# pangenome/impg

Measured on AMD Instinct MI355X. Metric: projected ranges/sec, 1M-PAF 100k-BED -x depth 3; CPU coitrees baseline, higher is better.
Workload: dtype int32

## Files before the change

### impg_amd/csrc/kernels.hip

```cpp
#include <hip/hip_runtime.h>

#include <cstring>
#include <type_traits>

#include "device_prims.hpp"
#include "impg_internal.hpp"
#include "kernels.hpp"

namespace impg {

__device__ __forceinline__ unsigned lane_id() { return threadIdx.x & 63u; }
__device__ __forceinline__ unsigned long long lanemask_lt() { return (1ull << lane_id()) - 1ull; }

template <int CTRL, int ROW_MASK>
__device__ __forceinline__ uint32_t dpp_or0(uint32_t x) {
  return (uint32_t)__builtin_amdgcn_update_dpp(0, (int)x, CTRL, ROW_MASK, 0xF, false);
}
__device__ __forceinline__ uint32_t wave_incl_scan(uint32_t x) {
  x += dpp_or0<0x111, 0xF>(x);
  x += dpp_or0<0x112, 0xF>(x);
  x += dpp_or0<0x114, 0xF>(x);
  x += dpp_or0<0x118, 0xF>(x);
  x += dpp_or0<0x142, 0xA>(x);
  x += dpp_or0<0x143, 0xC>(x);
// ... 2172 lines not shown
      const int sdir = reversed_entry ? 1 : (is_reverse ? -1 : 1);
      const int pdir = reversed_entry ? (is_reverse ? -1 : 1) : 1;
      const int32_t s0 = reversed_entry ? m_ts : (is_reverse ? m_te : m_ts);
      const int32_t p0 = reversed_entry ? (is_reverse ? m_qe : m_qs) : m_qs;
      const int64_t x_lo = sdir > 0 ? (int64_t)rs - s0 : (int64_t)s0 - re, x_hi = sdir > 0 ? (int64_t)re - s0 : (int64_t)s0 - rs;
      auto S = [&](uint32_t k) -> int64_t { const uint4 b = B[k]; return (int64_t)(reversed_entry ? b.y : b.x); };
      uint32_t lo = 1, hi = n + 1;
      while (lo < hi) { const uint32_t mid = (lo + hi) >> 1; if (S(mid) <= x_lo) lo = mid + 1; else hi = mid; }
      const uint32_t first = lo - 1;
      lo = 0; hi = n;
      while (lo < hi) { const uint32_t mid = (lo + hi) >> 1; if (S(mid) < x_hi) lo = mid + 1; else hi = mid; }
      if (first < n && lo > 0 && first <= lo - 1) {
        const uint32_t last = lo - 1;
        const uint4 bf0 = B[first], bf1 = B[first + 1], bl0 = B[last], bl1 = B[last + 1];
        auto seg = [&](const uint4 &a, const uint4 &b, int32_t &ppos, int32_t &pdelta, int32_t &sstart, int32_t &send, int32_t &asd) {
          const int32_t sa = (int32_t)(reversed_entry ? a.y : a.x), sb = (int32_t)(reversed_entry ? b.y : b.x);
          const int32_t ja = (int32_t)(reversed_entry ? a.x : a.y), jb = (int32_t)(reversed_entry ? b.x : b.y);
          const int32_t pa = s0 + sdir * sa, pb = s0 + sdir * sb;
          sstart = min(pa, pb); send = max(pa, pb); asd = sb - sa;
          ppos = p0 + pdir * ja; pdelta = pdir * (jb - ja);
        };
        const int32_t qlo = min(m_qs, m_qe), qhi = max(m_qs, m_qe);
        int32_t ppos, pdelta, sstart, send, asd;
        seg(bf0, bf1, ppos, pdelta, sstart, send, asd);
        const int32_t refined_first = tp_refine(ppos, pdelta, sstart, max(sstart, rs), asd, true, qlo, qhi);
        seg(bl0, bl1, ppos, pdelta, sstart, send, asd);
        const int32_t refined_last = tp_refine(ppos, pdelta, sstart, min(send, re), asd, false, qlo, qhi);
        bool keep = true;
        int64_t mm = 0, xx = 0;
        if (CIGAR || use_ident) { mm = (int64_t)bl1.z - bf0.z; xx = (int64_t)bl1.w - bf0.w; }
        if (use_ident) {
          const int64_t total = mm + xx;
          const double ident = total == 0 ? 0.0 : (double)mm / (double)total;
          keep = !(ident < min_identity);
        }
        if (keep) {
          if (refined_first < 0 || refined_last < 0) atomicOr(err_flag, 2u);
          const bool swap_q = is_reverse && !reversed_entry;
          out = make_int4(swap_q ? refined_last : refined_first, swap_q ? refined_first : refined_last, rs, re);
          qid = e1.x;
          ok = true;
          if (CIGAR) {
            const bool fits = mm <= (int64_t)OP_LEN_MASK && xx <= (int64_t)OP_LEN_MASK;
            if (!fits) atomicOr(err_flag, 4u);
            sl.a[p] = (uint32_t)mm;
            sl.off[p] = (int32_t)xx;
            sl.n[p] = fits ? (mm > 0 ? 1u : 0u) + (xx > 0 ? 1u : 0u) : 0u;
            sl.rem[p] = 0;
          }
        }
      }
    }
    h.qid[p] = qid;
    if (ok) h.c[p] = out;
  }
  __shared__ uint32_t wcnt[4];
  unsigned long long m = __ballot(ok);
  if (lane_id() == 0) wcnt[threadIdx.x >> 6] = __popcll(m);
  __syncthreads();
  if (threadIdx.x == 0) {
    uint32_t tot = wcnt[0] + wcnt[1] + wcnt[2] + wcnt[3];
    if (tot) atomicAdd(&accepted[(blockIdx.x % COUNT_SLOTS) * COUNT_STRIDE], (unsigned long long)tot);
  }
}

__global__ __launch_bounds__(256) void slice_counts_kernel(HitArrays h, SliceArrays sl, uint32_t n_pairs,
                                                           uint32_t *__restrict__ cnt) {
  const uint32_t p = blockIdx.x * 256u + threadIdx.x;
  if (p >= n_pairs) return;
  cnt[p] = h.qid[p] == HIT_NONE ? 0u : sl.n[p];
}
__global__ __launch_bounds__(64) void slice_write_kernel(DeviceIndexView v, const uint32_t *__restrict__ pair_entry,
                                                         HitArrays h, SliceArrays sl, uint32_t n_pairs,
                                                         const uint32_t *__restrict__ off, uint32_t *__restrict__ out) {
  const uint32_t p = blockIdx.x * 64u + threadIdx.x;
  if (p >= n_pairs || h.qid[p] == HIT_NONE) return;
  const Entry &en = v.entries[pair_entry[p]];
  const bool swp = (en.nops_flags & EF_REVERSED) != 0, flip = swp && (en.nops_flags & EF_STRAND);
  const uint32_t *rec = v.ops + (size_t)en.tile_base * TILE_WORDS;
  const uint32_t n = sl.n[p], a = sl.a[p];
  uint32_t *o = out + off[p];
  for (uint32_t t = 0; t < n; t++) {
    const uint32_t oi = flip ? a - t : a + t;
    uint32_t op = rec[(size_t)(oi / TILE_OPS) * TILE_WORDS + 6 + oi % TILE_OPS];
    if (swp) {
      const uint32_t code = op >> 29;
      if (code == 2u) op = (3u << 29) | (op & OP_LEN_MASK);
      else if (code == 3u) op = (2u << 29) | (op & OP_LEN_MASK);
    }
    o[t] = op;
  }
  const int32_t fo = sl.off[p], lr = sl.rem[p];
  if (fo > 0) o[0] = (o[0] & (7u << 29)) | (uint32_t)((int32_t)(o[0] & OP_LEN_MASK) - fo);
  if (lr < 0) o[n - 1] = (o[n - 1] & (7u << 29)) | (uint32_t)((int32_t)(o[n - 1] & OP_LEN_MASK) + lr);
}

__global__ __launch_bounds__(256) void slice_write_tp_kernel(HitArrays h, SliceArrays sl, uint32_t n_pairs,
                                                             const uint32_t *__restrict__ off, uint32_t *__restrict__ out) {
  const uint32_t p = blockIdx.x * 256u + threadIdx.x;
  if (p >= n_pairs || h.qid[p] == HIT_NONE || sl.n[p] == 0u) return;
  const uint32_t mm = sl.a[p], xx = (uint32_t)sl.off[p];
  uint32_t *o = out + off[p];
  if (mm) *o++ = mm | (0u << 29);
  if (xx) *o = xx | (1u << 29);
}

__device__ __forceinline__ unsigned long long mix64(unsigned long long z) {
  z = (z ^ (z >> 30)) * 0xBF58476D1CE4E5B9ull;
  z = (z ^ (z >> 27)) * 0x94D049BB133111EBull;
  return z ^ (z >> 31);
}
__global__ __launch_bounds__(256) void hit_stats_kernel(const FrontierRec *__restrict__ fr,
                                                        const uint32_t *__restrict__ pair_range, uint32_t n_pairs,
                                                        HitArrays h, int32_t min_output_length, int skip_same_target,
                                                        unsigned long long *__restrict__ rstat, int want_ck, uint32_t stride) {
  const uint32_t p = blockIdx.x * 256u + threadIdx.x;
  uint32_t r = 0xFFFFFFFFu;
  unsigned long long c = 0, a = 0;
  if (p < n_pairs) {
    r = pair_range[(size_t)p * stride];
    const uint32_t qid = h.qid[(size_t)p * stride];
    if (qid != HIT_NONE) {
      const uint32_t tgt = fr[r].target_id;
      const int4 hc = h.c[p];
      const int32_t qs = hc.x, qe = hc.y;
      const bool drop = (min_output_length >= 0 && abs(qe - qs) < min_output_length) ||
                        (skip_same_target && qid == tgt);
      if (!drop) {
        if (want_ck) {
          a = mix64(((unsigned long long)qid << 32) | (uint32_t)qs);
          a = mix64(a ^ (((unsigned long long)(uint32_t)qe << 32) | tgt));
          a = mix64(a ^ (((unsigned long long)(uint32_t)hc.z << 32) | (uint32_t)hc.w));
        }
        c = 1;
      }
    }
  }
  const unsigned lane = lane_id();
  const uint32_t prev = (uint32_t)__shfl_up((int)r, 1);
  const unsigned long long heads = __ballot(lane == 0 || prev != r);
  if (__popcll(heads) < 64) {
    const unsigned first = 63u - (unsigned)__clzll((long long)(heads & (lanemask_lt() | (1ull << lane))));
#pragma unroll
    for (unsigned o = 1; o < 64; o <<= 1) {
      const unsigned long long cv = (unsigned long long)__shfl_up((long long)c, o);
      const unsigned long long av = (unsigned long long)__shfl_up((long long)a, o);
      if (lane >= first + o) { c += cv; a += av; }
    }
  }
  const bool tail = lane == 63u || ((heads >> (lane + 1u)) & 1ull);
  if (tail && c && r != 0xFFFFFFFFu) {
    atomicAdd(&rstat[2u * (size_t)r], c);
    if (want_ck) atomicAdd(&rstat[2u * (size_t)r + 1u], a);
  }
}
__global__ __launch_bounds__(256) void range_stats_reduce_kernel(const FrontierRec *__restrict__ fr, uint32_t n_fr,
                                                                 const unsigned long long *__restrict__ rstat,
                                                                 unsigned long long *__restrict__ count,
                                                                 unsigned long long *__restrict__ cksum) {
  const uint32_t i = blockIdx.x * 256u + threadIdx.x;
  uint32_t q = 0xFFFFFFFFu;
  unsigned long long c = 0, a = 0;
  if (i < n_fr) {
    q = fr[i].qidx;
    const ulonglong2 x = reinterpret_cast<const ulonglong2 *>(rstat)[i];
    c = x.x; a = x.y;
  }
  const unsigned lane = lane_id();
  const uint32_t prev = (uint32_t)__shfl_up((int)q, 1);
  const unsigned long long heads = __ballot(lane == 0 || prev != q);
  const unsigned first = 63u - (unsigned)__clzll((long long)(heads & (lanemask_lt() | (1ull << lane))));
#pragma unroll
  for (unsigned o = 1; o < 64; o <<= 1) {
    const unsigned long long cv = (unsigned long long)__shfl_up((long long)c, o);
    const unsigned long long av = (unsigned long long)__shfl_up((long long)a, o);
    if (lane >= first + o) { c += cv; a += av; }
  }
  const bool tail = lane == 63u || ((heads >> (lane + 1u)) & 1ull);
  if (tail && q != 0xFFFFFFFFu && (c | a)) {
    if (count && c) atomicAdd(&count[q], c);
    if (cksum && a) atomicAdd(&cksum[q], a);
  }
}

__global__ __launch_bounds__(256) void update_keys_kernel(const FrontierRec *__restrict__ fr,
                                                          const uint32_t *__restrict__ pair_range, uint32_t n_pairs,
                                                          HitArrays h, unsigned long long *__restrict__ keys,
                                                          unsigned long long *__restrict__ vals,
                                                          unsigned long long *__restrict__ n_active) {
  const uint32_t p = blockIdx.x * 256u + threadIdx.x;
  unsigned long long k = ~0ull;
  if (p < n_pairs) {
    const uint32_t qid = h.qid[p];
    unsigned long long v = 0;
    if (qid != HIT_NONE) {
      const FrontierRec f = fr[pair_range[p]];
      if (qid != f.target_id) {
        k = ((unsigned long long)f.qidx << 32) | qid;
        const int4 hc = h.c[p];
        v = ((unsigned long long)(uint32_t)min(hc.x, hc.y) << 32) | (uint32_t)max(hc.x, hc.y);
      }
    }
    keys[p] = k;
    vals[p] = v;
  }
  __shared__ uint32_t wcnt[4];
  unsigned long long m = __ballot(k != ~0ull);
  if (lane_id() == 0) wcnt[threadIdx.x >> 6] = __popcll(m);
  __syncthreads();
  if (threadIdx.x == 0) {
    uint32_t tot = wcnt[0] + wcnt[1] + wcnt[2] + wcnt[3];
    if (tot) atomicAdd(&n_active[(blockIdx.x % COUNT_SLOTS) * COUNT_STRIDE], (unsigned long long)tot);
  }
}

__global__ __launch_bounds__(256) void group_heads_kernel(const unsigned long long *__restrict__ skeys, uint32_t n,
                                                          uint32_t *__restrict__ head) {
  const uint32_t i = blockIdx.x * 256u + threadIdx.x;
  if (i >= n) return;
  const unsigned long long k = skeys[i];
  head[i] = (k != ~0ull) && (i == 0 || skeys[i - 1] != k);
}
__global__ __launch_bounds__(256) void group_scatter_kernel(const unsigned long long *__restrict__ skeys, uint32_t n,
                                                            const uint32_t *__restrict__ head,
                                                            const uint32_t *__restrict__ gid,
                                                            uint32_t *__restrict__ gstart,
                                                            unsigned long long *__restrict__ gkey) {
  const uint32_t i = blockIdx.x * 256u + threadIdx.x;
  if (i >= n) return;
  if (head[i]) {
    gstart[gid[i]] = i;
    gkey[gid[i]] = skeys[i];
  }
}

constexpr uint32_t GROUP_ITEMS = 8, GROUP_TILE = 256u * GROUP_ITEMS;
__global__ __launch_bounds__(256) void group_count_kernel(const unsigned long long *__restrict__ skeys, uint32_t n, uint32_t *__restrict__ tile_heads) {
  const uint32_t base = blockIdx.x * GROUP_TILE + threadIdx.x * GROUP_ITEMS;
  unsigned long long prev = base > 0 && base <= n ? skeys[base - 1u] : 0ull;
  uint32_t c = 0;
#pragma unroll
  for (uint32_t k = 0; k < GROUP_ITEMS; k++) {
    const uint32_t i = base + k;
    const unsigned long long key = i < n ? skeys[i] : ~0ull;
    c += (key != ~0ull && (i == 0 || key != prev)) ? 1u : 0u;
    prev = key;
  }
  uint32_t tot;
  block_excl_scan(c, &tot);
  if (threadIdx.x == 0) tile_heads[blockIdx.x] = tot;
}
__global__ __launch_bounds__(256) void group_fill_kernel(const unsigned long long *__restrict__ skeys, uint32_t n, const uint32_t *__restrict__ tile_base,
                                                         uint32_t *__restrict__ gstart, unsigned long long *__restrict__ gkey) {
  const uint32_t base = blockIdx.x * GROUP_TILE + threadIdx.x * GROUP_ITEMS;
  unsigned long long key[GROUP_ITEMS];
  unsigned long long prev = base > 0 && base <= n ? skeys[base - 1u] : 0ull;
  uint32_t c = 0, flags = 0;
#pragma unroll
  for (uint32_t k = 0; k < GROUP_ITEMS; k++) {
    const uint32_t i = base + k;
    key[k] = i < n ? skeys[i] : ~0ull;
    if (key[k] != ~0ull && (i == 0 || key[k] != prev)) { flags |= 1u << k; c += 1u; }
    prev = key[k];
  }
  uint32_t tot;
  uint32_t g = tile_base[blockIdx.x] + block_excl_scan(c, &tot);
#pragma unroll
  for (uint32_t k = 0; k < GROUP_ITEMS; k++)
    if (flags & (1u << k)) { gstart[g] = base + k; gkey[g] = key[k]; g += 1u; }
}

constexpr uint32_t SEG_MAX_SEQ = 2048, SEG_WAVES = 4;
constexpr uint32_t SEG_BIG_QUERY = 32768;
constexpr uint32_t SEG_SLICE_HITS = 8192, SEG_BIG_SLICE = 131072, SEG_MAX_PARTS = 4096;
__global__ __launch_bounds__(256) void run_bounds_kernel(const uint32_t *__restrict__ pair_range, uint32_t n, uint32_t *__restrict__ run_start,
                                                         uint32_t *__restrict__ run_end) {
  const uint32_t p = blockIdx.x * 256u + threadIdx.x;
  if (p >= n) return;
  const uint32_t r = pair_range[p];
  if (p == 0 || pair_range[p - 1u] != r) run_start[r] = p;
  if (p + 1u == n || pair_range[p + 1u] != r) run_end[r] = p + 1u;
}
__global__ __launch_bounds__(256) void run_bounds_by_offsets_kernel(const uint32_t *__restrict__ perm, const uint32_t *__restrict__ pair_off,
                                                                    const uint32_t *__restrict__ cnt, uint32_t n_fr,
                                                                    uint32_t *__restrict__ run_start, uint32_t *__restrict__ run_end) {
  const uint32_t i = blockIdx.x * 256u + threadIdx.x;
  if (i >= n_fr) return;
  const uint32_t r = perm ? perm[i] : i, a = pair_off[i];
  run_start[r] = a;
  run_end[r] = a + cnt[i];
}
__global__ __launch_bounds__(256) void query_bounds_kernel(const FrontierRec *__restrict__ fr, uint32_t n_fr, uint32_t n_queries, uint32_t *__restrict__ qfirst,
                                                           uint32_t *__restrict__ qlast, uint32_t *__restrict__ unsorted) {
  const uint32_t i = blockIdx.x * 256u + threadIdx.x;
  if (i >= n_fr) return;
  const uint32_t q = fr[i].qidx;
  if (q >= n_queries) { *unsorted = 1u; return; }
  if (i == 0 || fr[i - 1u].qidx != q) {
    qfirst[q] = i;
    if (i && fr[i - 1u].qidx > q) *unsorted = 1u;
  }
  if (i + 1u == n_fr || fr[i + 1u].qidx != q) qlast[q] = i + 1u;
}
template <bool WITH_HC, class F>
__device__ __forceinline__ void seg_for_chunks(const FrontierRec *__restrict__ fr, const uint32_t *__restrict__ run_start,
                                               const uint32_t *__restrict__ run_end, const HitArrays &h, uint32_t f0, uint32_t f1, F f) {
  const uint32_t lane = lane_id();
  for (uint32_t base = f0; base < f1; base += 64u) {
    const uint32_t i = base + lane;
    const bool have = i < f1;
    const uint32_t rs = have ? run_start[i] : 0u, re = have ? run_end[i] : 0u, tg = have ? fr[i].target_id : 0u;
    const uint32_t m = min(64u, f1 - base);
    uint32_t j = 0, c0 = 0, e = 0, t = 0;
    auto seek = [&](uint32_t &jj, uint32_t &cc, uint32_t &ee, uint32_t &tt) {
      while (jj < m && cc >= ee) {
        jj += 1u;
        if (jj < m) {
          cc = (uint32_t)__builtin_amdgcn_readlane((int)rs, (int)jj);
          ee = (uint32_t)__builtin_amdgcn_readlane((int)re, (int)jj);
          tt = (uint32_t)__builtin_amdgcn_readlane((int)tg, (int)jj);
        }
      }
    };
    c0 = (uint32_t)__builtin_amdgcn_readlane((int)rs, 0);
    e = (uint32_t)__builtin_amdgcn_readlane((int)re, 0);
    t = (uint32_t)__builtin_amdgcn_readlane((int)tg, 0);
    seek(j, c0, e, t);
    uint32_t qid = HIT_NONE;
    int4 hc = make_int4(0, 0, 0, 0);
    if (j < m && c0 + lane < e) { qid = h.qid[c0 + lane]; if (WITH_HC) hc = h.c[c0 + lane]; }
    while (j < m) {
      uint32_t nj = j, nc = c0 + 64u, ne = e, nt = t;
      seek(nj, nc, ne, nt);
      uint32_t nqid = HIT_NONE;
      int4 nhc = make_int4(0, 0, 0, 0);
      if (nj < m && nc + lane < ne) { nqid = h.qid[nc + lane]; if (WITH_HC) nhc = h.c[nc + lane]; }
      f(qid, hc, qid != HIT_NONE && qid != t);
      j = nj; c0 = nc; e = ne; t = nt; qid = nqid; hc = nhc;
    }
  }
}
template <bool COUNT_ONLY>
__global__ __launch_bounds__(64 * SEG_WAVES) void seg_group_kernel(const FrontierRec *__restrict__ fr, const uint32_t *__restrict__ qfirst,
                                                                   const uint32_t *__restrict__ qlast, const uint32_t *__restrict__ run_start,
                                                                   const uint32_t *__restrict__ run_end, HitArrays h, uint32_t n_queries, uint32_t nb,
                                                                   uint32_t nbits, uint32_t *__restrict__ qact, const uint32_t *__restrict__ qdst,
                                                                   uint32_t *__restrict__ qgrp, const uint32_t *__restrict__ gdst,
                                                                   uint32_t *__restrict__ gstart, unsigned long long *__restrict__ gkey,
                                                                   unsigned long long *__restrict__ svals, uint32_t *__restrict__ qbins,
                                                                   uint32_t parts, uint32_t *__restrict__ qtot) {
  extern __shared__ __attribute__((aligned(16))) uint32_t seg_bins[];
  const uint32_t w = threadIdx.x >> 6, lane = lane_id();
  const uint32_t u = blockIdx.x * SEG_WAVES + w;
  if (u >= n_queries * parts) return;
  const bool sliced = parts > 1u;
  const uint32_t q = sliced ? u / parts : u, part = u - q * parts;
  uint32_t f0 = qfirst[q], f1 = qlast[q];
  if (sliced) {
    const uint32_t len = f1 > f0 ? f1 - f0 : 0u;
    f1 = f0 + (uint32_t)(((unsigned long long)len * (part + 1u)) / parts);
    f0 = f0 + (uint32_t)(((unsigned long long)len * part) / parts);
  } else if (f0 >= f1) { if (COUNT_ONLY && lane == 0) { qact[q] = 0u; qgrp[q] = 0u; } return; }
  uint32_t *bins = seg_bins + w * nb;
  if (COUNT_ONLY || !qbins) {
    for (uint32_t b = lane; b < nb; b += 64u) bins[b] = 0u;
    __builtin_amdgcn_wave_barrier();
    seg_for_chunks<false>(fr, run_start, run_end, h, f0, f1, [&](uint32_t qid, const int4 &, bool active) { if (active) atomicAdd(&bins[qid], 1u); });
  } else if (!sliced) {
    for (uint32_t b = lane; b < nb; b += 64u) bins[b] = qbins[(size_t)q * nb + b];
  }
  __builtin_amdgcn_wave_barrier();
  if (COUNT_ONLY) {
    uint32_t cnt = 0, grp = 0;
    for (uint32_t b = lane; b < nb; b += 64u) {
      const uint32_t x = bins[b];
      cnt += x; grp += x ? 1u : 0u;
      if (qbins) qbins[(size_t)u * nb + b] = x;
    }
#pragma unroll
    for (int o = 32; o > 0; o >>= 1) { cnt += (uint32_t)__shfl_xor((int)cnt, o); grp += (uint32_t)__shfl_xor((int)grp, o); }
    if (lane == 0) {
      if (!sliced) { qact[q] = cnt; qgrp[q] = grp; }
      if (cnt > (sliced ? SEG_BIG_SLICE : SEG_BIG_QUERY)) atomicMax(qact + 4u * (size_t)n_queries + 1u, cnt);
    }
    return;
  }
  const uint32_t dst0 = qdst[q];
  const unsigned long long khi = (unsigned long long)q << 32;
  uint32_t carry = 0, g = gdst[q];
  for (uint32_t b = 0; b < nb; b += 64u) {
    const uint32_t x = sliced ? qtot[(size_t)q * nb + b + lane] : bins[b + lane];
    const uint32_t inc = wave_incl_scan(x);
    const uint32_t off = carry + inc - x;
    bins[b + lane] = off + (sliced ? qbins[(size_t)u * nb + b + lane] : 0u);
    carry += (uint32_t)__builtin_amdgcn_readlane((int)inc, 63);
    const unsigned long long gm = __ballot(x != 0u);
    if (x && part == 0u) {
      const uint32_t gi = g + (uint32_t)__popcll(gm & lanemask_lt());
      gstart[gi] = dst0 + off;
      gkey[gi] = khi | (b + lane);
    }
    g += (uint32_t)__popcll(gm);
  }
  __builtin_amdgcn_wave_barrier();
  seg_for_chunks<true>(fr, run_start, run_end, h, f0, f1, [&](uint32_t qid, const int4 &hc, bool active) {
    const unsigned long long am = __ballot(active);
    if (!am) return;
    unsigned long long mask = am;
    for (uint32_t b = 0; b < nbits; b++) {
      const bool bit = (qid >> b) & 1u;
      const unsigned long long bal = __ballot(active && bit);
      mask &= bit ? bal : ~bal;
    }
    if (active) {
      const uint32_t pos = dst0 + bins[qid] + (uint32_t)__popcll(mask & lanemask_lt());
      svals[pos] = ((unsigned long long)(uint32_t)min(hc.x, hc.y) << 32) | (uint32_t)max(hc.x, hc.y);
    }
    __builtin_amdgcn_wave_barrier();
    if (active && lane == 63u - (uint32_t)__clzll((long long)mask)) bins[qid] += (uint32_t)__popcll(mask);
    __builtin_amdgcn_wave_barrier();
  });
}

__global__ __launch_bounds__(256) void seg_parts_scan_kernel(uint32_t *__restrict__ qbins, uint32_t nb, uint32_t parts, uint32_t *__restrict__ qtot,
                                                             uint32_t *__restrict__ qact, uint32_t *__restrict__ qgrp) {
  const uint32_t q = blockIdx.x, b = blockIdx.y * 256u + threadIdx.x;
  uint32_t run = 0;
  if (b < nb) {
    uint32_t *p = qbins + (size_t)q * parts * nb + b;
    uint32_t k = 0;
    for (; k + 4u <= parts; k += 4u) {
      const uint32_t x0 = p[(size_t)k * nb], x1 = p[(size_t)(k + 1u) * nb], x2 = p[(size_t)(k + 2u) * nb], x3 = p[(size_t)(k + 3u) * nb];
      p[(size_t)k * nb] = run; run += x0;
      p[(size_t)(k + 1u) * nb] = run; run += x1;
      p[(size_t)(k + 2u) * nb] = run; run += x2;
      p[(size_t)(k + 3u) * nb] = run; run += x3;
    }
    for (; k < parts; k++) { const uint32_t x = p[(size_t)k * nb]; p[(size_t)k * nb] = run; run += x; }
    qtot[(size_t)q * nb + b] = run;
  }
  uint32_t cnt = run, grp = run ? 1u : 0u;
#pragma unroll
  for (int o = 32; o > 0; o >>= 1) { cnt += (uint32_t)__shfl_xor((int)cnt, o); grp += (uint32_t)__shfl_xor((int)grp, o); }
  if (lane_id() == 0 && cnt) { atomicAdd(&qact[q], cnt); atomicAdd(&qgrp[q], grp); }
}

__device__ __forceinline__ uint32_t lower_bound_u64(const unsigned long long *a, uint32_t n, unsigned long long k) {
  uint32_t lo = 0, hi = n;
  while (lo < hi) {
    uint32_t mid = (lo + hi) >> 1;
    if (a[mid] < k) lo = mid + 1; else hi = mid;
  }
  return lo;
}

__global__ __launch_bounds__(256) void table_qoff_kernel(const unsigned long long *__restrict__ keys, uint32_t n_groups, uint32_t n_queries,
                                                         uint32_t *__restrict__ qoff) {
  const uint32_t q = blockIdx.x * 256u + threadIdx.x;
  if (q <= n_queries) qoff[q] = lower_bound_u64(keys, n_groups, (unsigned long long)q << 32);
}
__global__ __launch_bounds__(256) void group_prepare_kernel(VisitedTables vt, const unsigned long long *__restrict__ gkey,
                                                            const uint32_t *__restrict__ gstart, uint32_t n_groups,
                                                            uint32_t n_active, uint32_t *__restrict__ glen,
                                                            const int2 **__restrict__ old_src,
                                                            uint32_t *__restrict__ cap, uint32_t *__restrict__ pcap) {
  const uint32_t g = blockIdx.x * 256u + threadIdx.x;
  if (g >= n_groups) return;
  const uint32_t st = gstart[g];
  const uint32_t en = g + 1 < n_groups ? gstart[g + 1] : n_active;
  const uint32_t len = en - st;
  glen[g] = len;
  const unsigned long long k = gkey[g];
  const int2 *src = nullptr;
  uint32_t olen = 0;
  bool found = false;
  const uint32_t q = (uint32_t)(k >> 32);
  for (int t = (int)vt.n_tables - 1; t >= 0; t--) {
    const VisitedTable &T = vt.t[t];
    const uint32_t lo = T.qoff[q], hi = T.qoff[q + 1u];
    const uint32_t i = lo + lower_bound_u64(T.keys + lo, hi - lo, k);
    if (i < hi && T.keys[i] == k) {
      src = T.ranges + T.off[i];
      olen = T.len[i];
      found = true;
      break;
    }
  }
  if (!found && vt.mask_off) {
    const uint32_t seq = (uint32_t)(k & 0xFFFFFFFFull);
    const uint32_t a = vt.mask_off[seq];
    olen = vt.mask_off[seq + 1] - a;
    src = vt.mask_ranges + a;
  }
  old_src[g] = olen ? src : nullptr;
  cap[g] = olen + len;
  pcap[g] = olen + 2u * len;
}

__device__ __forceinline__ uint32_t lower_bound_start(const int2 *a, uint32_t n, int32_t s) {
  uint32_t lo = 0, hi = n;
  while (lo < hi) {
    uint32_t mid = (lo + hi) >> 1;
    if (a[mid].x < s) lo = mid + 1; else hi = mid;
  }
  return lo;
}

#ifndef IMPG_VU_LDS_CAP
#define IMPG_VU_LDS_CAP 12
#endif
constexpr uint32_t VU_LDS_CAP = IMPG_VU_LDS_CAP;
#ifndef IMPG_VW_TINY
#define IMPG_VW_TINY 192
#endif
#ifndef IMPG_VW_SMALL
#define IMPG_VW_SMALL 1152
#endif
#ifndef IMPG_VU_TINY_MAX
#define IMPG_VU_TINY_MAX 12
#endif
#ifndef IMPG_VU_MID_MAX
#define IMPG_VU_MID_MAX 48
#endif
#ifndef IMPG_VU_MID_CAP
#define IMPG_VU_MID_CAP 64
#endif
constexpr uint32_t VU_TINY_MAX = IMPG_VU_TINY_MAX, VU_MID_MAX = IMPG_VU_MID_MAX, VU_MID_CAP = IMPG_VU_MID_CAP;
static_assert(VU_TINY_MAX <= VU_LDS_CAP && VU_MID_MAX <= VU_MID_CAP, "a lane's list must fit its LDS column");
constexpr uint32_t VW_CAP_TINY = IMPG_VW_TINY, VW_CAP_SMALL = IMPG_VW_SMALL, VW_CAP_LARGE = 4096,
                   VW_SMALL_HEADROOM = 256;
struct ListInPlace {
  int2 *p;
  __device__ __forceinline__ int32_t &x(uint32_t i) const { return p[i].x; }
  __device__ __forceinline__ int32_t &y(uint32_t i) const { return p[i].y; }
};
struct ListInLds {
  int32_t *bx, *by;
  __device__ __forceinline__ int32_t &x(uint32_t i) const { return bx[i * 64u]; }
  __device__ __forceinline__ int32_t &y(uint32_t i) const { return by[i * 64u]; }
};
template <class L> __device__ __forceinline__ uint32_t list_lower_bound(const L &R, uint32_t n, int32_t s) {
  uint32_t lo = 0, hi = n;
  while (lo < hi) {
    const uint32_t mid = (lo + hi) >> 1;
    if (R.x(mid) < s) lo = mid + 1; else hi = mid;
  }
  return lo;
}
template <class L, class E, class G>
__device__ __forceinline__ void replay_one(const L &R, uint32_t &len, int32_t start, int32_t end, int32_t sequence_length,
                                           int32_t min_transitive_len, int32_t mdbr, E &&emit, G &&grow) {
  bool should_add = true;
  if (mdbr > 0) {
    const uint32_t idx = list_lower_bound(R, len, start);
    if (idx > 0 && abs(start - R.y(idx - 1)) < mdbr) should_add = false;
    if (should_add && idx < len && abs(R.x(idx) - end) < mdbr) should_add = false;
  }
  if (!should_add) return;
  if (start < 0) start = 0;
  if (end > sequence_length) end = sequence_length;
  int32_t current = start;
  const uint32_t pos = list_lower_bound(R, len, start);
  uint32_t i = pos;
  if (i > 0 && R.y(i - 1) > start) i -= 1;
  while (i < len && current < end) {
    const int32_t rx = R.x(i), ry = R.y(i);
    if (rx > end) break;
    if (current < rx) {
      if (abs(rx - current) >= min_transitive_len) emit(current, rx);
    }
    current = max(current, ry);
    i += 1;
  }
  if (current < end) {
    if (abs(end - current) >= min_transitive_len) emit(current, end);
  }
  uint32_t mfrom;
  if (pos > 0 && R.y(pos - 1) >= start) {
    R.y(pos - 1) = max(R.y(pos - 1), end);
    mfrom = pos - 1;
  } else if (pos < len && end >= R.x(pos)) {
    R.x(pos) = min(start, R.x(pos));
    R.y(pos) = max(end, R.y(pos));
    mfrom = pos;
  } else {
    grow();
    for (uint32_t k = len; k > pos; k--) { R.x(k) = R.x(k - 1); R.y(k) = R.y(k - 1); }
    R.x(pos) = start;
    R.y(pos) = end;
    len += 1;
    return;
  }
  uint32_t write = mfrom, read = mfrom + 1;
  while (read < len) {
    if (R.y(write) >= R.x(read)) {
      R.y(write) = max(R.y(write), R.y(read));
    } else {
      write += 1;
      const int32_t tx = R.x(write), ty = R.y(write);
      R.x(write) = R.x(read); R.y(write) = R.y(read);
      R.x(read) = tx; R.y(read) = ty;
    }
    read += 1;
  }
  len = write + 1;
}
template <class L>
__device__ __forceinline__ uint32_t replay_hits(const L &R, uint32_t len, const unsigned long long *__restrict__ svals,
                                                uint32_t st, uint32_t n, int32_t sequence_length,
                                                int32_t min_transitive_len, int32_t mdbr, int2 *__restrict__ P, uint32_t &np) {
  for (uint32_t t = 0; t < n; t++) {
    const unsigned long long iv = svals[st + t];
    replay_one(R, len, (int32_t)(uint32_t)(iv >> 32), (int32_t)(uint32_t)iv, sequence_length, min_transitive_len, mdbr,
               [&](int32_t a, int32_t b) { P[np++] = make_int2(a, b); }, [] {});
  }
  return len;
}
#ifdef IMPG_VU_CLOCKS
constexpr uint32_t VU_CLK_ROWS = 1024;
__device__ unsigned long long g_vu_clk[VU_CLK_ROWS][16];
#define VU_MARK(i) do { asm volatile("s_waitcnt vmcnt(0) lgkmcnt(0)" ::: "memory"); vu_t[i] = __builtin_readcyclecounter(); } while (0)
#else
#define VU_MARK(i) do { } while (0)
#endif
typedef const unsigned long long __attribute__((address_space(1))) *global_list_t;
__device__ __forceinline__ int2 list_range(global_list_t p, uint32_t i) {
  const unsigned long long v = p[i];
  return make_int2((int32_t)(uint32_t)v, (int32_t)(uint32_t)(v >> 32));
}
#ifndef IMPG_VU_WAVES
#define IMPG_VU_WAVES 6
#endif
#pragma clang diagnostic push
#pragma clang diagnostic ignored "-Wpass-failed"
template <uint32_t CAP, bool LISTED>
__global__ __launch_bounds__(64) __attribute__((amdgpu_waves_per_eu(IMPG_VU_WAVES, IMPG_VU_WAVES)))
void visited_update_kernel(const unsigned long long *__restrict__ svals,
                                                            const int32_t *__restrict__ seq_len,
                                                            const unsigned long long *__restrict__ gkey,
                                                            const uint32_t *__restrict__ gstart,
                                                            const uint32_t *__restrict__ glen,
                                                            const unsigned long long *__restrict__ old_src,
                                                            const uint32_t *__restrict__ cap,
                                                            const uint32_t *__restrict__ noff,
                                                            const uint32_t *__restrict__ poff, uint32_t n_groups,
                                                            int32_t min_transitive_len, int32_t mdbr,
                                                            int2 *__restrict__ new_ranges, uint32_t *__restrict__ new_len,
                                                            int2 *__restrict__ pieces, uint32_t *__restrict__ n_pieces,
                                                            const uint32_t *__restrict__ list, const uint32_t *__restrict__ n_list,
                                                            uint32_t *__restrict__ reach) {
  __shared__ int32_t lds_x[CAP * 64], lds_y[CAP * 64];
  const uint32_t n_items = LISTED ? *n_list : n_groups;
  for (uint32_t item0 = blockIdx.x * 64u; item0 < n_items; item0 += gridDim.x * 64u) {
  const uint32_t item = item0 + threadIdx.x;
#ifdef IMPG_VU_CLOCKS
  unsigned long long vu_t[8];
  VU_MARK(0);
#endif
  const bool have = item < n_items;
  const uint32_t g = LISTED ? list[min(item, n_items - 1u)] : item;
  const uint32_t gi = min(g, n_groups - 1u);
  const uint32_t c_ = cap[gi], n_ = glen[gi], st_ = gstart[gi], no = noff[gi], po = poff[gi];
  const global_list_t src_ = (global_list_t)old_src[gi];
  const unsigned long long key = gkey[gi];
  const uint32_t c = have ? c_ : 0u;
  const bool mine = have && (LISTED || c <= VU_TINY_MAX);
  const uint32_t n = mine ? n_ : 0u, st = mine ? st_ : 0u;
  const uint32_t olen = mine ? c - n : 0u;
  int2 *R = new_ranges + no;
  int2 *P = pieces + po;
  VU_MARK(1);
  const int32_t sequence_length = seq_len[(uint32_t)(key & 0xFFFFFFFFull)];
  const unsigned long long *hp = svals + st;
  const uint32_t hl = max(n, 1u) - 1u;
  unsigned long long h0 = hp[0], h1 = hp[min(1u, hl)], h2 = hp[min(2u, hl)], h3 = hp[min(3u, hl)];
  const global_list_t src = olen ? src_ : (global_list_t)(unsigned long long)(uintptr_t)svals;
  const uint32_t sl = max(olen, 1u) - 1u;
  const int2 s0 = list_range(src, 0), s1 = list_range(src, min(1u, sl)), s2 = list_range(src, min(2u, sl)), s3 = list_range(src, min(3u, sl));
  VU_MARK(2);
  uint32_t len = olen, np = 0;
  VU_MARK(3);
  const bool fast = mine;
  const ListInLds A{lds_x + threadIdx.x, lds_y + threadIdx.x};
  if (fast) {
    if (olen > 0) { A.x(0) = s0.x; A.y(0) = s0.y; }
    if (olen > 1) { A.x(1) = s1.x; A.y(1) = s1.y; }
    if (olen > 2) { A.x(2) = s2.x; A.y(2) = s2.y; }
    if (olen > 3) { A.x(3) = s3.x; A.y(3) = s3.y; }
    for (uint32_t i = 4; i < olen; i += 4) {
      const uint32_t l = olen - 1u;
      const int2 r0 = list_range(src, i), r1 = list_range(src, min(i + 1u, l)), r2 = list_range(src, min(i + 2u, l)), r3 = list_range(src, min(i + 3u, l));
      A.x(i) = r0.x; A.y(i) = r0.y;
      if (i + 1u < olen) { A.x(i + 1u) = r1.x; A.y(i + 1u) = r1.y; }
      if (i + 2u < olen) { A.x(i + 2u) = r2.x; A.y(i + 2u) = r2.y; }
      if (i + 3u < olen) { A.x(i + 3u) = r3.x; A.y(i + 3u) = r3.y; }
    }
  }
  VU_MARK(4);
  const uint32_t nf = fast ? n : 0u;
  const uint32_t nmax = wave_max_u32(nf);
  bool spilled = false;
  auto spill = [&]() {
    for (uint32_t k = 0; k < np; k++) P[k] = make_int2(A.x(CAP - 1u - k), A.y(CAP - 1u - k));
    spilled = true;
  };
  auto emit = [&](int32_t a, int32_t b) {
    if (!spilled && len + np >= CAP) spill();
    if (!spilled) { A.x(CAP - 1u - np) = a; A.y(CAP - 1u - np) = b; }
// ... 2141 lines not shown
```

Baseline: 76.97 billion.

## Flatten run chunks via wave prefix scan and batch hit fetches in seg_for_chunks

Replaces the per-run readlane seek loop with a wave-wide prefix scan over run lengths. Each lane then binary-searches the scan to find its run, so a 64-run window is processed as a dense stream of hits. Loads are unrolled four wide with double buffering, and the next window's run bounds are prefetched. Hit coordinates are read as int2 instead of int4, which halves that traffic. The cost is more shuffles per fetch and higher register pressure. Runs shorter than 64 no longer waste whole wave iterations.

```diff
diff --git a/impg_amd/csrc/kernels.hip b/impg_amd/csrc/kernels.hip
--- a/impg_amd/csrc/kernels.hip
+++ b/impg_amd/csrc/kernels.hip
@@ -2498,41 +2498,55 @@
   }
   if (i + 1u == n_fr || fr[i + 1u].qidx != q) qlast[q] = i + 1u;
 }
+constexpr uint32_t SEG_U = 4;
+__device__ __forceinline__ uint32_t wave_read(uint32_t x, uint32_t src_lane) { return (uint32_t)__shfl((int)x, (int)src_lane); }
 template <bool WITH_HC, class F>
 __device__ __forceinline__ void seg_for_chunks(const FrontierRec *__restrict__ fr, const uint32_t *__restrict__ run_start,
                                                const uint32_t *__restrict__ run_end, const HitArrays &h, uint32_t f0, uint32_t f1, F f) {
   const uint32_t lane = lane_id();
-  for (uint32_t base = f0; base < f1; base += 64u) {
+  auto load_base = [&](uint32_t base, uint32_t &rs, uint32_t &re, uint32_t &tg) {
     const uint32_t i = base + lane;
     const bool have = i < f1;
-    const uint32_t rs = have ? run_start[i] : 0u, re = have ? run_end[i] : 0u, tg = have ? fr[i].target_id : 0u;
-    const uint32_t m = min(64u, f1 - base);
-    uint32_t j = 0, c0 = 0, e = 0, t = 0;
-    auto seek = [&](uint32_t &jj, uint32_t &cc, uint32_t &ee, uint32_t &tt) {
-      while (jj < m && cc >= ee) {
-        jj += 1u;
-        if (jj < m) {
-          cc = (uint32_t)__builtin_amdgcn_readlane((int)rs, (int)jj);
-          ee = (uint32_t)__builtin_amdgcn_readlane((int)re, (int)jj);
-          tt = (uint32_t)__builtin_amdgcn_readlane((int)tg, (int)jj);
-        }
+    rs = have ? run_start[i] : 0u; re = have ? run_end[i] : 0u; tg = have ? fr[i].target_id : 0u;
+  };
+  uint32_t rs, re, tg;
+  load_base(f0, rs, re, tg);
+  for (uint32_t base = f0; base < f1; base += 64u) {
+    const uint32_t len = re > rs ? re - rs : 0u, incl = wave_incl_scan(len);
+    const uint32_t total = (uint32_t)__builtin_amdgcn_readlane((int)incl, 63);
+    const uint32_t first = rs - (incl - len), tgt = tg;
+    if (base + 64u < f1) load_base(base + 64u, rs, re, tg);
+    auto fetch = [&](uint32_t x0, uint32_t &qid, int2 &hc, uint32_t &t) {
+      qid = HIT_NONE; hc = make_int2(0, 0); t = 0u;
+      if (x0 >= total) return;
+      const uint32_t x = x0 + lane;
+      uint32_t j = 0;
+#pragma unroll
+      for (uint32_t s = 32u; s; s >>= 1) {
+        const uint32_t v = wave_read(incl, j + s - 1u);
+        j += v <= x ? s : 0u;
+      }
+      const uint32_t slot = wave_read(first, j) + x;
+      t = wave_read(tgt, j);
+      if (x < total) {
+        qid = h.qid[slot];
+        if (WITH_HC) hc = *reinterpret_cast<const int2 *>(h.c + slot);
       }
     };
-    c0 = (uint32_t)__builtin_amdgcn_readlane((int)rs, 0);
-    e = (uint32_t)__builtin_amdgcn_readlane((int)re, 0);
-    t = (uint32_t)__builtin_amdgcn_readlane((int)tg, 0);
-    seek(j, c0, e, t);
-    uint32_t qid = HIT_NONE;
-    int4 hc = make_int4(0, 0, 0, 0);
-    if (j < m && c0 + lane < e) { qid = h.qid[c0 + lane]; if (WITH_HC) hc = h.c[c0 + lane]; }
-    while (j < m) {
-      uint32_t nj = j, nc = c0 + 64u, ne = e, nt = t;
-      seek(nj, nc, ne, nt);
-      uint32_t nqid = HIT_NONE;
-      int4 nhc = make_int4(0, 0, 0, 0);
-      if (nj < m && nc + lane < ne) { nqid = h.qid[nc + lane]; if (WITH_HC) nhc = h.c[nc + lane]; }
-      f(qid, hc, qid != HIT_NONE && qid != t);
-      j = nj; c0 = nc; e = ne; t = nt; qid = nqid; hc = nhc;
+    uint32_t qid[SEG_U], t[SEG_U];
+    int2 hc[SEG_U];
+#pragma unroll
+    for (uint32_t u = 0; u < SEG_U; u++) fetch(64u * u, qid[u], hc[u], t[u]);
+    for (uint32_t x0 = 0; x0 < total; x0 += 64u * SEG_U) {
+      uint32_t nqid[SEG_U], nt[SEG_U];
+      int2 nhc[SEG_U];
+#pragma unroll
+      for (uint32_t u = 0; u < SEG_U; u++) fetch(x0 + 64u * (SEG_U + u), nqid[u], nhc[u], nt[u]);
+#pragma unroll
+      for (uint32_t u = 0; u < SEG_U; u++)
+        if (x0 + 64u * u < total) f(qid[u], hc[u], qid[u] != HIT_NONE && qid[u] != t[u]);
+#pragma unroll
+      for (uint32_t u = 0; u < SEG_U; u++) { qid[u] = nqid[u]; hc[u] = nhc[u]; t[u] = nt[u]; }
     }
   }
 }
@@ -2561,7 +2575,7 @@
   if (COUNT_ONLY || !qbins) {
     for (uint32_t b = lane; b < nb; b += 64u) bins[b] = 0u;
     __builtin_amdgcn_wave_barrier();
-    seg_for_chunks<false>(fr, run_start, run_end, h, f0, f1, [&](uint32_t qid, const int4 &, bool active) { if (active) atomicAdd(&bins[qid], 1u); });
+    seg_for_chunks<false>(fr, run_start, run_end, h, f0, f1, [&](uint32_t qid, const int2 &, bool active) { if (active) atomicAdd(&bins[qid], 1u); });
   } else if (!sliced) {
     for (uint32_t b = lane; b < nb; b += 64u) bins[b] = qbins[(size_t)q * nb + b];
   }
@@ -2599,7 +2613,7 @@
     g += (uint32_t)__popcll(gm);
   }
   __builtin_amdgcn_wave_barrier();
-  seg_for_chunks<true>(fr, run_start, run_end, h, f0, f1, [&](uint32_t qid, const int4 &hc, bool active) {
+  seg_for_chunks<true>(fr, run_start, run_end, h, f0, f1, [&](uint32_t qid, const int2 &hc, bool active) {
     const unsigned long long am = __ballot(active);
     if (!am) return;
     unsigned long long mask = am;
```

Result: faster. 78.12 billion (median of 6 runs) (+1.5%).
